# olivesgatech/R3D

Measured on AMD Instinct MI355X. Metric: training clips/sec (RGB+Depth fusion, DARai) at 1/2/4/8 GPUs; effective-rank match, higher is better.
Workload: dtype f32 (depth products: bf16x3 split on the bf16 matrix cores, fp32 accumulate)

## Files before the change

### include/r3d_hip.h

```cpp
#ifndef R3D_HIP_H
#define R3D_HIP_H

#include <stdint.h>

#ifdef __cplusplus
extern "C" {
#endif

#define R3D_ABI_VERSION 2

#define R3D_OK 0
#define R3D_EINVAL (-1)
#define R3D_EALIGN (-2)
#define R3D_ENORCCL (-3)
#define R3D_ERCCL_BASE (-100)

int r3d_abi_version(void);
int r3d_build_info(char* buf, int cap);

int r3d_allreduce_flat(float* buf, int64_t count, void* comm, void* stream);

#define R3D_GEMM_NT 0
#define R3D_GEMM_NN 1
#define R3D_GEMM_TN 2
// ... 97 lines not shown
    const float* q; int32_t ldq; const float* k; int32_t ldk; const float* v; int32_t ldv;
    const uint8_t* key_padding_mask; const int64_t* key_label; int32_t pad_idx;
    float* probs; const uint8_t* drop_mask; float drop_scale; float* o; int32_t ldo;
    int32_t B, heads, Lq, Lk, dh;
} r3d_mha_job;
int r3d_gemm_ln_mha_supported(int heads, int Lq, int Lk, int dh);
int r3d_gemm_ln_mha_fwd(const r3d_gemm_ln_job* jobs, int njobs, int H, const r3d_mha_job* mha, void* stream);

typedef struct r3d_fuser_chain_fwd_args {
    const float* x0; const float* h1;
    const float* wv; const float* wproj; const float* bproj; const float* g2; const float* be2;
    const float* w1; const float* b1; const float* w2; const float* b2; const float* gf; const float* bef;
    const float* pos; const float* wkv; const float* bkv; const float* wseg; const float* bseg;
    float* vsw; float* x1; float* h2; float* m2; float* r2; float* u; float* f1; float* x3; float* y; float* mf; float* rf;
    float* fused; float* seg; float* cakv;
    const float* qpos; const float* w_in; const float* b_in; const float* w_out; const float* b_out; const float* g1;
    const float* be1; const float* wq; const float* bq;
    const uint8_t* drop_sa; const uint8_t* drop_d1; float drop_scale;
    float* sa_qkv; float* p_sa; float* sa_o; float* t1_pre; float* t1; float* m1; float* r1; float* caq;
    int32_t N, S, K, H, add_xres, B, Q, heads;
    uint64_t* timeline;
    const uint16_t* pl_wv; const uint16_t* pl_wproj; const uint16_t* pl_w1; const uint16_t* pl_w2; const uint16_t* pl_wkv;
    const uint16_t* pl_wseg;
} r3d_fuser_chain_fwd_args;
typedef struct r3d_plane_job {
    const float* src; uint16_t* dst; int32_t ld, N, K, transposed, first_block, pad_;
} r3d_plane_job;
int64_t r3d_weight_plane_elems(int N, int K);
int r3d_weight_planes(const r3d_plane_job* jobs_device, int njobs, int total_blocks, void* stream);
int r3d_fuser_chain_supported(int N, int H, int K, int B, int Q, int heads);
int r3d_fuser_chain_fwd(const r3d_fuser_chain_fwd_args* a, void* stream);
typedef struct r3d_fuser_chain_bwd_args {
    const float* d_cakv; const float* d_seg; const float* d_extra; const float* wkv; const float* wseg;
    const float* x3; const float* mf; const float* rf; const float* gf;
    const float* w2; const float* u; const float* w1; const float* x1; const float* m2; const float* r2; const float* g2;
    const float* wproj; const float* wv; const float* x0; const float* m1; const float* r1; const float* g1n;
    const uint8_t* drop_x0; const float* m_rgb; const float* m_dep; const float* rgb; const float* dep_pre;
    const float* mean_d; const float* rstd_d; const float* lnd_g; const float* lnd_b;
    float* d_fused; float* d_x3; float* d_u; float* d_h2; float* d_x1; float* d_v; float* d_h1; float* d_rgb_pre;
    float* d_dep_pre; float* part_nf; float* part_n2; float* part_n1; float* part_dep;
    const float* d_caq; const float* d_t1_res; const float* wq; const float* t1_pre; const float* m1d; const float* r1d;
    const float* g1d; const uint8_t* drop_d1; const float* w_out; const float* sa_qkv; const float* p_sa;
    const uint8_t* drop_sa; const float* w_in;
    float* caqin; float* t1pre_out; float* sap; float* sao; float* saqkv; float* sain; float* part_d1;
    float drop_scale;
    int32_t N, S, K, H, add_xres, B, Q, heads;
// ... 200 lines not shown
```

### r3d_amd/_lib.py

```python
import ctypes as C
import os

HERE = os.path.dirname(os.path.abspath(__file__))
LIB_PATH = os.path.join(HERE, "_build", "libr3d_hip.so")
ABI_VERSION = 2

c_float_p = C.c_void_p


class GemmDesc(C.Structure):
    _fields_ = [
        ("A", C.c_void_p), ("B", C.c_void_p), ("C", C.c_void_p),
        ("layout", C.c_int32), ("M", C.c_int32), ("N", C.c_int32), ("K", C.c_int32),
        ("lda", C.c_int32), ("ldb", C.c_int32), ("ldc", C.c_int32),
        ("a_add", C.c_void_p), ("a_add_mod", C.c_int32), ("a_add_ld", C.c_int32), ("a_row_xor", C.c_int32),
        ("b_add", C.c_void_p), ("b_add_mod", C.c_int32), ("b_add_ld", C.c_int32),
        ("bias", C.c_void_p),
        ("pre_out", C.c_void_p), ("ldpre", C.c_int32),
        ("act", C.c_int32),
        ("drop_mask", C.c_void_p), ("lddrop", C.c_int32), ("drop_scale", C.c_float),
        ("aux", C.c_void_p), ("ldaux", C.c_int32), ("mul", C.c_int32),
        ("res1", C.c_void_p), ("ldr1", C.c_int32),
        ("res2", C.c_void_p), ("ldr2", C.c_int32),
        ("alpha", C.c_float), ("accumulate", C.c_int32),
# ... 21 lines not shown
                ("beta", C.c_void_p), ("relu", C.c_int32), ("add1", C.c_void_p), ("ldadd1", C.c_int32), ("add2", C.c_void_p),
                ("ldadd2", C.c_int32), ("dx", C.c_void_p), ("lddx", C.c_int32), ("dx2", C.c_void_p), ("lddx2", C.c_int32),
                ("drop_mask", C.c_void_p), ("lddrop", C.c_int32), ("drop_scale", C.c_float), ("dgamma", C.c_void_p),
                ("dbeta", C.c_void_p), ("ws", C.c_void_p), ("rows", C.c_int32), ("H", C.c_int32),
                ("rows_per_block", C.c_int32), ("nblocks", C.c_int32)]


class GemmLnJob(C.Structure):
    _fields_ = [("A", C.c_void_p), ("lda", C.c_int32), ("W", C.c_void_p), ("ldw", C.c_int32), ("bias", C.c_void_p),
                ("drop_mask", C.c_void_p), ("lddrop", C.c_int32), ("drop_scale", C.c_float),
                ("res1", C.c_void_p), ("ldr1", C.c_int32), ("res2", C.c_void_p), ("ldr2", C.c_int32),
                ("pre_out", C.c_void_p), ("ldpre", C.c_int32), ("gamma", C.c_void_p), ("beta", C.c_void_p),
                ("y", C.c_void_p), ("ldy", C.c_int32), ("mean", C.c_void_p), ("rstd", C.c_void_p),
                ("pair_out", C.c_void_p), ("M", C.c_int32), ("K", C.c_int32)]


class FuserChainFwdArgs(C.Structure):
    _PTRS = ("x0 h1 wv wproj bproj g2 be2 w1 b1 w2 b2 gf bef pos wkv bkv wseg bseg vsw x1 h2 m2 r2 u f1 x3 y mf rf fused seg "
             "cakv qpos w_in b_in w_out b_out g1 be1 wq bq drop_sa drop_d1").split()
    _PTRS2 = "sa_qkv p_sa sa_o t1_pre t1 m1 r1 caq".split()
    _PLANES = "pl_wv pl_wproj pl_w1 pl_w2 pl_wkv pl_wseg".split()
    _fields_ = ([(n, C.c_void_p) for n in _PTRS] + [("drop_scale", C.c_float)] + [(n, C.c_void_p) for n in _PTRS2] +
                [(n, C.c_int32) for n in "N S K H add_xres B Q heads".split()] + [("timeline", C.c_void_p)] +
                [(n, C.c_void_p) for n in _PLANES])


class PlaneJob(C.Structure):
    _fields_ = [("src", C.c_void_p), ("dst", C.c_void_p), ("ld", C.c_int32), ("N", C.c_int32), ("K", C.c_int32),
                ("transposed", C.c_int32), ("first_block", C.c_int32), ("pad_", C.c_int32)]


class FuserChainBwdArgs(C.Structure):
    _PTRS = ("d_cakv d_seg d_extra wkv wseg x3 mf rf gf w2 u w1 x1 m2 r2 g2 wproj wv x0 m1 r1 g1n drop_x0 m_rgb m_dep rgb "
             "dep_pre mean_d rstd_d lnd_g lnd_b d_fused d_x3 d_u d_h2 d_x1 d_v d_h1 d_rgb_pre d_dep_pre part_nf part_n2 "
             "part_n1 part_dep d_caq d_t1_res wq t1_pre m1d r1d g1d drop_d1 w_out sa_qkv p_sa drop_sa w_in caqin t1pre_out "
             "sap sao saqkv sain part_d1").split()
    _PLANES = "pl_wkv_t pl_wseg_t pl_w2_t pl_w1_t pl_wproj_t pl_wv_t".split()
    _fields_ = ([(n, C.c_void_p) for n in _PTRS] + [("drop_scale", C.c_float)] +
                [(n, C.c_int32) for n in "N S K H add_xres B Q heads".split()] + [("timeline", C.c_void_p)] +
                [(n, C.c_void_p) for n in _PLANES])


class DecoderChainArgs(C.Structure):
    _PTRS = ("caq cakv key_label p_ca drop_ca ca_o wo bo drop_d2 t1 t2_pre g2 be2 t2 m2 r2 w1 b1 drop_ff ff1 w2 b2 drop_d3 "
             "t3_pre d_t3pre d_ff2 d_ff1 d_t2pre d_cap d_cao d_caq d_cakv part_d2").split()
    _fields_ = ([(n, C.c_void_p) for n in _PTRS] + [("drop_scale", C.c_float)] +
                [(n, C.c_int32) for n in "pad_idx B S H Q heads phases".split()] + [("timeline", C.c_void_p)] +
# ... 208 lines not shown
```

### r3d_amd/csrc/chain_common.h

```cpp
#pragma once
#include "common.h"

namespace r3d {

#define R3D_CHAIN_MARK(TL, WG_OK, K) do { if ((TL) && (WG_OK) && threadIdx.x == 0) (TL)[(K)] = wall_clock64(); } while (0)

struct FcMaskSrc {
    const uint8_t* p; size_t ld; bool on;
    __device__ __forceinline__ FcMaskSrc(const uint8_t* m, const void* fallback, size_t ld_)
        : p(m ? m : reinterpret_cast<const uint8_t*>(fallback)), ld(m ? ld_ : 0), on(m != nullptr) {}
    __device__ __forceinline__ uint8_t raw(size_t row, int col) const { return p[row * ld + (on ? col : 0)]; }
    __device__ __forceinline__ float keep(uint8_t b, float scale) const { return on ? scale * (float)b : 1.f; }
};

typedef float f32x4 __attribute__((ext_vector_type(4)));

constexpr int kFcH = 128;
constexpr int kFcRows = 16;
constexpr int kFcP1 = kFcH + 4;
constexpr int kFcP4 = 4 * kFcH + 4;
constexpr int kFcWP = kFcH + 4;
constexpr float kFcEps = 1e-5f;
__device__ __forceinline__ float fc_row16_sum(float v) {
    v += dpp_mov_f<0x128>(v);
// ... 107 lines not shown
#pragma unroll
    for (int i = 0; i < NR; ++i) { sa[i] = fc_row16_sum(a[i]); sb[i] = fc_row16_sum(b[i]); }
    if (li == 0) {
#pragma unroll
        for (int i = 0; i < NR; ++i) {
            red[(0 * 8 + wave) * kFcRows + NR * q + i] = sa[i];
            red[(1 * 8 + wave) * kFcRows + NR * q + i] = sb[i];
        }
    }
    __syncthreads();
#pragma unroll
    for (int i = 0; i < NR; ++i) {
        float x = 0.f, y = 0.f;
#pragma unroll
        for (int w8 = 0; w8 < 8; ++w8) {
            x += red[(0 * 8 + w8) * kFcRows + NR * q + i];
            y += red[(1 * 8 + w8) * kFcRows + NR * q + i];
        }
        sa[i] = x * (1.0f / (float)kFcH);
        sb[i] = y * (1.0f / (float)kFcH);
    }
}

}
```

### r3d_amd/csrc/fuser_chain.hip

```cpp
#include "chain_bf3.h"
#include "mha_small.h"
#include "../../include/r3d_hip.h"

namespace r3d {

constexpr int kFcBufH = 0;
constexpr int kFcBufV = kFcBufH + kFcRows * kFcP1;
constexpr int kFcBufF = kFcBufV + kFcRows * kFcP1;
constexpr int kFcWl = kFcBufF + kFcRows * kFcP4;
constexpr int kFcRed = kFcWl + 8 * 16 * kFcWP;
constexpr int kFcLdsFloats = kFcRed + 2 * 8 * kFcRows;
constexpr int kFcLdsBytes = kFcLdsFloats * 4;
static_assert(mha_small_lds_floats(16, 8) <= 16 * kFcWP, "the query role's attention units borrow the wave's weight region");
static_assert(mha_small_bwd_lds_floats(16, 8) <= 16 * kFcWP, "the query role's attention units borrow the wave's weight region");

typedef r3d_fuser_chain_fwd_args FcFwd;

__device__ __forceinline__ void fc_fwd_fuser(const FcFwd& A, const int wg, float* lds) {
    const int tid = threadIdx.x, lane = tid & 63, wave = tid >> 6;
    const int li = lane & 15, q = lane >> 4;
    float* bufH = lds + kFcBufH;
    float* bufV = lds + kFcBufV;
    float* bufF = lds + kFcBufF;
    float* wl = lds + kFcWl + wave * (16 * kFcWP);
// ... 307 lines not shown
        const int r = 4 * q + i;
        const float t1 = (t1p[i] - mean[i]) * rstd[i] * g1 + be1;
        A.t1[(size_t)(row0 + r) * H + c] = t1;
        bufH[r * kFcP1 + c] = t1 + qp[i];
        if (wave == 0 && li == 0) { A.m1[row0 + r] = mean[i]; A.r1[row0 + r] = rstd[i]; }
    }
    __syncthreads();
    R3D_CHAIN_MARK(A.timeline, wgq == 0, 20);
    fc_opload(a, bufH + li * kFcP1 + 4 * q);
    acc0 = zero; acc1 = zero;
    fc_chunk(a, wr, acc0, acc1);
#pragma unroll
    for (int i = 0; i < 4; ++i) A.caq[(size_t)(row0 + 4 * q + i) * H + c] = (acc0[i] + acc1[i]) + b_q;
    R3D_CHAIN_MARK(A.timeline, wgq == 0, 21);
}

constexpr int kF3P1 = kFcH + 8;
constexpr int kF3P4 = 4 * kFcH + 8;
constexpr int kF3ImgH = 0;
constexpr int kF3ImgV = kF3ImgH + 3 * 16 * kF3P1;
constexpr int kF3ImgF = kF3ImgV + 3 * 16 * kF3P1;
constexpr int kF3RedBytes = (kF3ImgF + 3 * 16 * kF3P4) * 2;
constexpr int kF3LdsBytes = kF3RedBytes + 2 * 2 * 8 * kFcRows * 4;

__device__ __forceinline__ void fc3_fwd_fuser(const FcFwd& A, const int wg, float* lds) {
    const int tid = threadIdx.x, lane = tid & 63, wave = tid >> 6;
    const int li = lane & 15, q = lane >> 4;
    unsigned short* img = reinterpret_cast<unsigned short*>(lds);
    unsigned short* imgH = img + kF3ImgH;
    unsigned short* imgV = img + kF3ImgV;
    unsigned short* imgF = img + kF3ImgF;
    float (*red)[8][kFcRows] = reinterpret_cast<float (*)[8][kFcRows]>(reinterpret_cast<unsigned char*>(lds) + kF3RedBytes);
    const int row0 = wg * kFcRows;
    const int c = wave * 16 + li;
    constexpr int H = kFcH;
    const int nseg_t = (A.K + 15) >> 4;
    const bool has12 = wave < nseg_t;
    R3D_CHAIN_MARK(A.timeline, wg == 0, 0);
    Bf3B b0, b1, b2;
    bf3_bload<4>(b0, A.pl_wv, 4, wave, 0, lane);
    bf3_bload<4>(b1, A.pl_wproj, 4, wave, 0, lane);
    bf3_bload<4>(b2, A.pl_w1, 4, 4 * wave + 0, 0, lane);
    const f32x4 a_in = *reinterpret_cast<const f32x4*>(A.h1 + (size_t)(row0 + (tid >> 5)) * H + 4 * (tid & 31));
    float x0[4];
#pragma unroll
    for (int i = 0; i < 4; ++i) x0[i] = A.x0[(size_t)(row0 + 4 * q + i) * H + c];
// ... 120 lines not shown
    acc0 = zero; acc1 = zero;
    bf3_chunk<4>(imgV, kF3P1, li, q, 0, b1, acc0, acc1);
    if (q >= 2) {
#pragma unroll
        for (int i = 0; i < 4; ++i) A.cakv[(size_t)(fr + i) * (2 * H) + wave * 16 + li] = (acc0[i] + acc1[i]) + bkv0;
    }
    acc0 = zero; acc1 = zero;
    bf3_chunk<4>(imgV, kF3P1, li, q, 0, b2, acc0, acc1);
    if (q >= 2) {
#pragma unroll
        for (int i = 0; i < 4; ++i) A.cakv[(size_t)(fr + i) * (2 * H) + (wave + 8) * 16 + li] = (acc0[i] + acc1[i]) + bkv1;
    }
    if (has12) {
        acc0 = zero; acc1 = zero;
        bf3_chunk<4>(imgV, kF3P1, li, q, 0, b0, acc0, acc1);
        if (q < 2 && cseg < A.K) {
#pragma unroll
            for (int i = 0; i < 4; ++i) A.seg[(size_t)(fr + i) * A.K + cseg] = (acc0[i] + acc1[i]) + bsg;
        }
    }
    R3D_CHAIN_MARK(A.timeline, wg == 0, 7);
}

__global__ __launch_bounds__(512) void fuser_chain_fwd_bf3_kernel(const FcFwd A) {
    extern __shared__ __attribute__((aligned(16))) float lds[];
    if (threadIdx.x >= 256) __builtin_amdgcn_s_setprio(0); else __builtin_amdgcn_s_setprio(2);
    const int nf = (2 * A.N) / kFcRows;
    if ((int)blockIdx.x < nf) fc3_fwd_fuser(A, (int)blockIdx.x, lds);
    else fc_fwd_query(A, (int)blockIdx.x - nf, lds);
}

__global__ __launch_bounds__(256) void weight_planes_kernel(const r3d_plane_job* __restrict__ jobs, int njobs, int total) {
    weight_planes_block(jobs, njobs, total, (int)blockIdx.x * 4 + (threadIdx.x >> 6), threadIdx.x & 63);
}

__global__ __launch_bounds__(512) void fuser_chain_fwd_kernel(const FcFwd A) {
    extern __shared__ __attribute__((aligned(16))) float lds[];
    if (threadIdx.x >= 256) __builtin_amdgcn_s_setprio(0); else __builtin_amdgcn_s_setprio(2);
    const int nf = (2 * A.N) / kFcRows;
    if ((int)blockIdx.x < nf) fc_fwd_fuser(A, (int)blockIdx.x, lds);
    else fc_fwd_query(A, (int)blockIdx.x - nf, lds);
}


constexpr int kFbWl = kFcBufF + kFcRows * kFcP4;
constexpr int kFbRed = kFbWl + 8 * 128 * kFbWP;
constexpr int kFbLdsFloats = kFbRed + 2 * 2 * 8 * kFcRows;
constexpr int kFbLdsBytes = kFbLdsFloats * 4;
static_assert(mha_small_bwd_lds_floats(16, 8) <= 128 * kFbWP, "attention units borrow the wave's weight region");
static_assert(kFbLdsBytes <= 160 * 1024, "LDS");

typedef r3d_fuser_chain_bwd_args FcBwd;
// ... 636 lines not shown

R3D_EXPORT int r3d_fuser_chain_supported(int N, int H, int K, int B, int Q, int heads) {
    return (H == r3d::kFcH && N > 0 && (2 * N) % r3d::kFcRows == 0 && K > 0 && K <= 128 && B > 0 && Q == 8 && heads == 8 &&
            (B * Q) % r3d::kFcRows == 0) ? 1 : 0;
}

R3D_EXPORT int r3d_fuser_chain_fwd(const r3d_fuser_chain_fwd_args* a, void* stream) {
    R3D_REQUIRE(a);
    R3D_REQUIRE(r3d_fuser_chain_supported(a->N, a->H, a->K, a->B, a->Q, a->heads));
    R3D_REQUIRE(a->S > 0 && a->N % a->S == 0);
    R3D_REQUIRE(a->x0 && a->h1 && a->wv && a->wproj && a->bproj && a->g2 && a->be2 && a->w1 && a->b1 && a->w2 && a->b2 && a->gf &&
                a->bef && a->pos && a->wkv && a->bkv && a->wseg && a->bseg);
    R3D_REQUIRE(a->vsw && a->x1 && a->h2 && a->m2 && a->r2 && a->u && a->f1 && a->x3 && a->mf && a->rf && a->fused && a->seg &&
                a->cakv);
    R3D_REQUIRE(a->qpos && a->w_in && a->b_in && a->w_out && a->b_out && a->g1 && a->be1 && a->wq && a->bq);
    R3D_REQUIRE(a->sa_qkv && a->p_sa && a->sa_o && a->t1_pre && a->t1 && a->m1 && a->r1 && a->caq);
    const void* al[] = {a->h1, a->wv, a->wproj, a->w1, a->w2, a->wkv, a->wseg, a->qpos, a->w_in, a->w_out, a->wq, a->sa_o,
                        a->sa_qkv};
    for (const void* p : al)
        if (!r3d_aligned16(p)) return R3D_EALIGN;
    hipError_t e = hipFuncSetAttribute((const void*)r3d::fuser_chain_fwd_kernel, hipFuncAttributeMaxDynamicSharedMemorySize,
                                       r3d::kFcLdsBytes);
    if (e != hipSuccess) return (int)e;
    const int grid = (2 * a->N) / r3d::kFcRows + (a->B * a->Q) / r3d::kFcRows;
    if (a->pl_wv) {
        R3D_REQUIRE(a->pl_wproj && a->pl_w1 && a->pl_w2 && a->pl_wkv && a->pl_wseg);
        const int ldsb = r3d::kFcLdsBytes > r3d::kF3LdsBytes ? r3d::kFcLdsBytes : r3d::kF3LdsBytes;
        e = hipFuncSetAttribute((const void*)r3d::fuser_chain_fwd_bf3_kernel, hipFuncAttributeMaxDynamicSharedMemorySize, ldsb);
        if (e != hipSuccess) return (int)e;
        hipLaunchKernelGGL(r3d::fuser_chain_fwd_bf3_kernel, dim3(grid), dim3(512), (size_t)ldsb, (hipStream_t)stream, *a);
        R3D_LAUNCH_CHECK();
        return R3D_OK;
    }
    hipLaunchKernelGGL(r3d::fuser_chain_fwd_kernel, dim3(grid), dim3(512), (size_t)r3d::kFcLdsBytes, (hipStream_t)stream, *a);
    R3D_LAUNCH_CHECK();
    return R3D_OK;
}

R3D_EXPORT int64_t r3d_weight_plane_elems(int N, int K) { return N > 0 && K > 0 ? (int64_t)r3d::bf3_plane_elems(N, K) : 0; }

R3D_EXPORT int r3d_weight_planes(const r3d_plane_job* jobs_device, int njobs, int total_blocks, void* stream) {
    R3D_REQUIRE(jobs_device && njobs > 0 && total_blocks > 0);
    hipLaunchKernelGGL(r3d::weight_planes_kernel, dim3(r3d_cdiv(total_blocks, 4)), dim3(256), 0, (hipStream_t)stream, jobs_device,
                       njobs, total_blocks);
    R3D_LAUNCH_CHECK();
    return R3D_OK;
}
// ... 33 lines not shown
```

### r3d_amd/engine.py

```python
import math

import torch

from . import ops
from ._lib import GEMM_NT, GEMM_NN, GEMM_TN

LIVE_PREFIXES = ("input_embed.", "depth_projection.", "depth_layernorm.", "pos_embedding", "query_embed.",
                 "fuser.blocks.", "fuser.norm.", "transformer.decoder.", "fc_seg.", "fc.", "fc_len.")
EXCLUDE_CLASS_IDX = 47
DROP_P = 0.1


BN_LIVE_PREFIXES = ("fuser.alpha", "fuser.bn_rgb.", "fuser.bn_depth.")
VARY_LIVE_PREFIXES = ("fuser.alpha",)


def is_live(name):
    return name.startswith(LIVE_PREFIXES)


BWD_BF3_MAX_K = 32


def fuser_chain_shape_ok(B, S, H, K, Q, heads, bn=False):
    return bool(not bn and H // heads == 16 and ops.fuser_chain_supported(B * S, H, K, B, Q, heads))


def decoder_chain_shape_ok(B, S, H, Q, heads, L):
    return bool(L == 1 and H // heads == 16 and B * Q <= 1024 and ops.decoder_chain_supported(H, Q, heads, S))


def bwd_chain_bf3(chain_bf3, K):
    return bool(chain_bf3 and K <= BWD_BF3_MAX_K)


def tail_in_decoder_chain(B, H, K, Q):
    return ops.tail_losses_supported(H, K + 1, Q, B * Q)


class ParamArena:

    def __init__(self, named_params, device, extra_live=()):
        named = list(named_params)
        self.is_live = lambda n: is_live(n) or (bool(extra_live) and n.startswith(tuple(extra_live)))
        live = [(n, p) for n, p in named if self.is_live(n)]
        dead = [(n, p) for n, p in named if not self.is_live(n)]

        def key(item):
# ... 51 lines not shown


class _Shape:

    def __init__(self, eng, B, S, train):
        dev, H, Q, K, L, heads = eng.device, eng.H, eng.Q, eng.K, eng.L, eng.heads
        N, BQ = B * S, B * Q
        f = lambda *s: torch.empty(*s, dtype=torch.float32, device=dev)
        self.B, self.S, self.N, self.BQ = B, S, N, BQ
        self.rgb, self.dep, self.dep_pre = f(N, H), f(N, H), f(N, H)
        self.mean_d, self.rstd_d = f(N), f(N)
        if eng.bn:
            self.bn_mean, self.bn_rstd, self.bn_absg = f(2, H), f(2, H), f(2, H)
            self.bn_idx = torch.empty(2, max(1, int(H * 0.1)), dtype=torch.int64, device=dev)
        self.no_xres = bool(eng.bn or eng.vary)
        self.sums = torch.empty(2, H, dtype=torch.float64, device=dev)
        self.idx = torch.empty(2, H // 4, dtype=torch.int64, device=dev)
        self.mask = f(2, H)
        self.x0, self.h1, self.vsw, self.x1, self.h2 = f(2 * N, H), f(2 * N, H), f(2 * N, H), f(2 * N, H), f(2 * N, H)
        self.u, self.f1 = f(2 * N, 4 * H), f(2 * N, 4 * H)
        self.x3, self.y = f(2 * N, H), f(2 * N, H)
        self.m1, self.r1, self.m2, self.r2, self.mf, self.rf = f(2 * N), f(2 * N), f(2 * N), f(2 * N), f(2 * N), f(2 * N)
        self.fused = f(N, H)
        self.tgt0 = torch.zeros(BQ, H, dtype=torch.float32, device=dev)
        self.layers = []
        for _ in range(L):
            d = dict(sa_qkv=f(BQ, 3 * H), sa_o=f(BQ, H), p_sa=f(B, heads, Q, Q), t1_pre=f(BQ, H),
                     t1=f(BQ, H), m1=f(BQ), r1=f(BQ), caq=f(BQ, H), cakv=f(N, 2 * H), ca_o=f(BQ, H),
                     p_ca=f(B, heads, Q, S), t2_pre=f(BQ, H), t2=f(BQ, H), m2=f(BQ), r2=f(BQ), ff1=f(BQ, 4 * H),
                     t3_pre=f(BQ, H), t3=f(BQ, H), m3=f(BQ), r3=f(BQ))
            self.layers.append(d)
        self.tgtF, self.mF, self.rF = f(BQ, H), f(BQ), f(BQ)
        self.actdur = f(BQ, K + 1)
        self.seg = f(N, K)
        self.loss = f(4)
        self.tables = {}
        self.loss_ws = torch.zeros(ops.losses_ws_floats(B, S, eng.Q), dtype=torch.float32, device=dev)
        self.counts = torch.zeros(4, dtype=torch.int64, device=dev)
        if train:
            self.d_actdur, self.d_seg = torch.zeros(BQ, K + 1, dtype=torch.float32, device=dev), f(N, K)
            self.d_tgtF, self.d_t = f(BQ, H), f(BQ, H)
            self.glayers = [dict(t3pre=f(BQ, H), ff2=f(BQ, H), ff1=f(BQ, 4 * H), t2=f(BQ, H), t2pre=f(BQ, H), cap=f(BQ, H),
                                 cao=f(BQ, H), caq=f(BQ, H), cakv=f(N, 2 * H), caqin=f(BQ, H), t1pre=f(BQ, H), sap=f(BQ, H),
                                 sao=f(BQ, H), saqkv=f(BQ, 3 * H), sain=f(BQ, H), t2b=f(BQ, H)) for _ in range(L)]
            self.d_fused, self.d_fused2 = f(N, H), f(N, H)
            lnw = lambda rows: f(max(ops.layernorm_bwd_ws_floats(rows, H), 4))
# ... 33 lines not shown
        self.pad_idx = module.src_pad_idx
        self.P, self.D = module.depth_projection.in_features, module.input_embed.in_features
        assert self.H % 8 == 0 and self.H % self.heads == 0
        self.bn = hasattr(module.fuser, "bn_rgb")
        self.vary = (not self.bn) and hasattr(module.fuser, "alpha")
        extra = BN_LIVE_PREFIXES if self.bn else (VARY_LIVE_PREFIXES if self.vary else ())
        self.arena = ParamArena(list(module.named_parameters()), self.device, extra)
        self.ws = ops.GemmWorkspace(self.device)
        self._sel = {}
        self.ws_side = ops.GemmWorkspace(self.device)
        self.side = torch.cuda.Stream(self.device)
        self.side2 = torch.cuda.Stream(self.device)
        self.ws_side2 = ops.GemmWorkspace(self.device)
        self.auto_side_stream = True
        self.use_side_stream = False
        self.use_fused_decoder = False
        self.use_fused_tail = True
        self.defer_tail = False
        self.use_paired_launches = True
        self.use_gemm_ln = True
        self.use_fuser_chain = True
        self.use_decoder_chain = True
        self.chain_bf3 = True
        self._planes = None
        self.overlap_planes = False
        self.overlap_param_tail = False
        self.ride_planes = True
        self._planes_rode = False
        self.fuse_depth_adamw = True
        self.pair_embeddings = True
        self._planes_forked = False
        self._tail_pending = False
        self._overlap_tail_now = False
        self.defer_loss_reduce = False
        self.loss_acc = None
        self.fold_rowsums = True
        self.ride_attention = True
        self.ride_attention_bwd = False
        self.split_k4h = False
        self.depth_prec = 1
        self.use_fused_embed = not (self.bn or self.vary)
        self.dropout_enabled = bool(getattr(module, "r3d_dropout_enabled", True))
        self.erank_weight = 0.0
        self.erank_warm_start = False
        self.erank_max_sweeps = 16
        self.erank_side_stream = True
# ... 337 lines not shown
                ent["pl_" + k] = (w_, False)
                ent["pl_" + k + "_t"] = (w_, True)
            self._planes = ops.WeightPlanes(ent, self.device)
        return self._planes

    def _multi_stream(self):
        return bool(self.use_side_stream or (self.auto_side_stream and self.H >= 512 and self.tp is None and
                                             self.grad_hook is None))

    def _planes_refresh(self):
        if self._planes_forked:
            torch.cuda.current_stream().wait_stream(self.side)
            self._planes_forked = False
        elif self._planes_rode:
            pass
        else:
            self.chain_planes().refresh()

    def _join_tail(self):
        if self._tail_pending:
            torch.cuda.current_stream().wait_stream(self.side)
            self._tail_pending = False

    def _chain_shape_ok(self, w):
        return fuser_chain_shape_ok(w.B, w.S, self.H, self.K, self.Q, self.heads, self.bn)

    def _chain_ok(self, w):
        return bool(self.use_fuser_chain and self._chain_shape_ok(w))

    def _dec_chain_ok(self, w):
        return bool(self.use_decoder_chain and decoder_chain_shape_ok(w.B, w.S, self.H, self.Q, self.heads, self.L))

    def _dec_chain(self, w, drop):
        bf3 = bool(self.chain_bf3)
        key = ("dec_chain", bool(drop), bf3)
        if bf3 and not (self.use_fuser_chain and self._chain_shape_ok(w)):
            self._planes_refresh()
        if key not in w.tables:
            pls = self.chain_planes() if bf3 else None
            dpl = None
            if pls is not None:
                dpl = dict(pl_wo=pls.ptr("pl_dec_wo"), pl_w1=pls.ptr("pl_dec_w1"), pl_w2=pls.ptr("pl_dec_w2"),
                           pl_w2_t=pls.ptr("pl_dec_w2_t"), pl_w1_t=pls.ptr("pl_dec_w1_t"), pl_wo_t=pls.ptr("pl_dec_wo_t"))
            a, H = self.arena, self.H
            c, pl = w.layers[0], "transformer.decoder.layers.0."
            dk = (lambda k: w.drop[k]) if drop else (lambda k: None)
# ... 17 lines not shown
        a, H, Q, S, B, BQ, heads, dh = self.arena, self.H, self.Q, w.S, w.B, w.BQ, self.heads, self.dh
        c, pl = w.layers[0], "transformer.decoder.layers.0."
        if self._chain_ok(w):
            bf3 = bool(self.chain_bf3)
            key = ("fwd_chain", bool(drop), bf3)
            if bf3:
                self._planes_refresh()
            if key not in w.tables:
                pls = self.chain_planes() if bf3 else None
                wi, bi = a.p(pl + "multihead_attn.in_proj_weight"), a.p(pl + "multihead_attn.in_proj_bias")
                w.tables[key] = ops.FuserChainFwd(
                    x0=w.x0, h1=w.h1, wv=wv, wproj=a.p(pre + "attn.proj.weight"), bproj=a.p(pre + "attn.proj.bias"),
                    g2=a.p(pre + "norm2.weight"), be2=a.p(pre + "norm2.bias"), w1=a.p(pre + "mlp.mlp.0.weight"),
                    b1=a.p(pre + "mlp.mlp.0.bias"), w2=a.p(pre + "mlp.mlp.2.weight"), b2=a.p(pre + "mlp.mlp.2.bias"),
                    gf=a.p("fuser.norm.weight"), bef=a.p("fuser.norm.bias"), pos=pos.contiguous(), wkv=wi[H:], bkv=bi[H:],
                    wseg=a.p("fc_seg.weight"), bseg=a.p("fc_seg.bias"), vsw=w.vsw, x1=w.x1, h2=w.h2, m2=w.m2, r2=w.r2, u=w.u,
                    f1=w.f1, x3=w.x3, y=w.y, mf=w.mf, rf=w.rf, fused=w.fused, seg=w.seg, cakv=c["cakv"],
                    qpos=qpos, w_in=a.p(pl + "self_attn.in_proj_weight"), b_in=a.p(pl + "self_attn.in_proj_bias"),
                    w_out=a.p(pl + "self_attn.out_proj.weight"), b_out=a.p(pl + "self_attn.out_proj.bias"),
                    g1=a.p(pl + "norm1.weight"), be1=a.p(pl + "norm1.bias"), wq=wi[:H], bq=bi[:H],
                    drop_sa=dm("sa_p0"), drop_d1=dm("d1_0"), drop_scale=dsc, sa_qkv=c["sa_qkv"], p_sa=c["p_sa"],
                    sa_o=c["sa_o"], t1_pre=c["t1_pre"], t1=c["t1"], m1=c["m1"], r1=c["r1"], caq=c["caq"],
                    N=w.N, S=S, K=self.K, H=H, add_xres=0 if w.no_xres else 1, B=B, Q=Q, heads=heads,
                    planes={k: pls.ptr(k) for k in pls.keys if not k.endswith("_t") and "dec_" not in k} if pls is not None else None)
            w.tables[key].launch()
            self._erank_fork(w)
            return
        key = ("fwd_pairs", bool(drop))
        if key not in w.tables:
            wi, bi = a.p(pl + "multihead_attn.in_proj_weight"), a.p(pl + "multihead_attn.in_proj_bias")
            t = 1 if H < 256 else 2
            g1 = ops.GemmGroup(GEMM_NT, [
                dict(a=w.h1, b=wv, c=w.vsw, c_row_xor=1),
                dict(a=w.tgt0, b=a.p(pl + "self_attn.in_proj_weight"), c=c["sa_qkv"], a_add=qpos, a_add_mod=Q,
                     bias=a.p(pl + "self_attn.in_proj_bias"))], tile=t)
            g2 = ops.GemmGroup(GEMM_NT, [
                dict(a=w.h2, b=a.p(pre + "mlp.mlp.0.weight"), c=w.f1, bias=a.p(pre + "mlp.mlp.0.bias"), act=2, pre_out=w.u),
                dict(a=c["sa_o"], b=a.p(pl + "self_attn.out_proj.weight"), c=c["t1_pre"],
                     bias=a.p(pl + "self_attn.out_proj.bias"), drop_mask=self._dm2(dm("d1_0"), BQ, H), drop_scale=dsc)],
                tile=t)
            g3 = ops.GemmGroup(GEMM_NT, [
                dict(a=w.fused, b=a.p("fc_seg.weight"), c=w.seg, bias=a.p("fc_seg.bias")),
                dict(a=w.fused, b=wi[H:], c=c["cakv"], bias=bi[H:], a_add=pos, a_add_mod=S),
                dict(a=c["t1"], b=wi[:H], c=c["caq"], a_add=qpos, a_add_mod=Q, bias=bi[:H])], tile=t)
            w.tables[key] = (g1, g2, g3)
        g1, g2, g3 = w.tables[key]
        g1.launch()
# ... 725 lines not shown
```

### r3d_amd/ops.py

```python
import ctypes as C

import torch

from . import _lib
from ._lib import GemmDesc, GEMM_NT, GEMM_NN, GEMM_TN, check


def _stream():
    return C.c_void_p(torch.cuda.current_stream().cuda_stream)


def _pv(t):
    return None if t is None else t.data_ptr()


def _p(t):
    if t is None:
        return None
    assert t.is_cuda, "r3d_amd kernels take device tensors only"
    return C.c_void_p(t.data_ptr())


def _f32(t, name="tensor"):
    assert t.dtype == torch.float32 and t.is_cuda, f"{name} must be a float32 device tensor"
# ... 342 lines not shown

    def refresh(self):
        check(_lib.load().r3d_weight_planes(_p(self.jobs_dev), self.njobs, self.blocks, _stream()), "r3d_weight_planes")

    def ptr(self, key):
        return self._ptr[key]

    def view(self, key):
        return self._view[key]


class FuserChainFwd:

    def __init__(self, **t):
        from ._lib import FuserChainFwdArgs
        a = FuserChainFwdArgs()
        dims = {k: t.pop(k) for k in ("N", "S", "K", "H", "add_xres", "B", "Q", "heads")}
        a.drop_scale = float(t.pop("drop_scale", 1.0))
        opt = {"y", "drop_sa", "drop_d1"}
        planes = t.pop("planes", None)
        if planes is not None:
            for name in FuserChainFwdArgs._PLANES:
                setattr(a, name, planes[name])
        for name in FuserChainFwdArgs._PTRS + FuserChainFwdArgs._PTRS2:
            v = t.pop(name, None)
            if v is None:
                assert name in opt, name
                continue
            assert v.is_cuda and v.is_contiguous(), name
            assert v.dtype == (torch.uint8 if name.startswith("drop_") else torch.float32), name
            setattr(a, name, v.data_ptr())
        assert not t, t.keys()
        for k, v in dims.items():
            setattr(a, k, int(v))
        self.args = a

    def launch(self):
        check(_lib.load().r3d_fuser_chain_fwd(C.byref(self.args), _stream()), "r3d_fuser_chain_fwd")


class FuserChainBwd:

    def __init__(self, **t):
        from ._lib import FuserChainBwdArgs
        a = FuserChainBwdArgs()
        dims = {k: t.pop(k) for k in ("N", "S", "K", "H", "add_xres", "B", "Q", "heads")}
# ... 604 lines not shown
```

Baseline: 44460.

## Split fuser-chain forward tiles across workgroup groups with last-arriver completion

When the tile grid leaves compute units idle, each 16-row fuser tile is split across 2 or 4 workgroups. Each workgroup computes its slice of the MLP hidden layer (w1) and publishes the bf16x3 planes to a global buffer. The last workgroup to arrive on an atomic counter then runs the w2 product, layernorm, fused and kv/seg outputs alone. This raises parallelism in the widest GEMM for small batches. In exchange it duplicates the early stages (v, proj, LN) in every group, adds global traffic for the packed planes, and adds an atomic handshake.

```diff
diff --git a/include/r3d_hip.h b/include/r3d_hip.h
--- a/include/r3d_hip.h
+++ b/include/r3d_hip.h
@@ -143,6 +143,7 @@
     uint64_t* timeline;
     const uint16_t* pl_wv; const uint16_t* pl_wproj; const uint16_t* pl_w1; const uint16_t* pl_w2; const uint16_t* pl_wkv;
     const uint16_t* pl_wseg;
+    int32_t groups; uint32_t* fc_count; uint64_t* fc_planes;
 } r3d_fuser_chain_fwd_args;
 typedef struct r3d_plane_job {
     const float* src; uint16_t* dst; int32_t ld, N, K, transposed, first_block, pad_;
diff --git a/r3d_amd/_lib.py b/r3d_amd/_lib.py
--- a/r3d_amd/_lib.py
+++ b/r3d_amd/_lib.py
@@ -67,7 +67,7 @@
     _PLANES = "pl_wv pl_wproj pl_w1 pl_w2 pl_wkv pl_wseg".split()
     _fields_ = ([(n, C.c_void_p) for n in _PTRS] + [("drop_scale", C.c_float)] + [(n, C.c_void_p) for n in _PTRS2] +
                 [(n, C.c_int32) for n in "N S K H add_xres B Q heads".split()] + [("timeline", C.c_void_p)] +
-                [(n, C.c_void_p) for n in _PLANES])
+                [(n, C.c_void_p) for n in _PLANES] + [("groups", C.c_int32), ("fc_count", C.c_void_p), ("fc_planes", C.c_void_p)])
 
 
 class PlaneJob(C.Structure):
diff --git a/r3d_amd/csrc/chain_common.h b/r3d_amd/csrc/chain_common.h
--- a/r3d_amd/csrc/chain_common.h
+++ b/r3d_amd/csrc/chain_common.h
@@ -153,4 +153,16 @@
     }
 }
 
+__device__ __forceinline__ bool fc_group_arrive(unsigned* count, int tile, int G, int* flag) {
+    asm volatile("s_waitcnt vmcnt(0)" ::: "memory");
+    __syncthreads();
+    if (threadIdx.x == 0)
+        *flag = (__hip_atomic_fetch_add(count + tile, 1u, __ATOMIC_RELAXED, __HIP_MEMORY_SCOPE_AGENT) == (unsigned)(G - 1)) ? 1 : 0;
+    __syncthreads();
+    return *flag != 0;
 }
+__device__ __forceinline__ void fc_group_reset(unsigned* count, int tile) {
+    if (threadIdx.x == 0) __hip_atomic_store(count + tile, 0u, __ATOMIC_RELAXED, __HIP_MEMORY_SCOPE_AGENT);
+}
+
+}
diff --git a/r3d_amd/csrc/fuser_chain.hip b/r3d_amd/csrc/fuser_chain.hip
--- a/r3d_amd/csrc/fuser_chain.hip
+++ b/r3d_amd/csrc/fuser_chain.hip
@@ -353,6 +353,7 @@
 constexpr int kF3ImgF = kF3ImgV + 3 * 16 * kF3P1;
 constexpr int kF3RedBytes = (kF3ImgF + 3 * 16 * kF3P4) * 2;
 constexpr int kF3LdsBytes = kF3RedBytes + 2 * 2 * 8 * kFcRows * 4;
+static_assert(kF3LdsBytes + 4 <= kFcLdsBytes, "the split's arrival flag sits behind the bf16x3 layout, inside the launch's LDS");
 
 __device__ __forceinline__ void fc3_fwd_fuser(const FcFwd& A, const int wg, float* lds) {
     const int tid = threadIdx.x, lane = tid & 63, wave = tid >> 6;
@@ -519,12 +520,203 @@
     R3D_CHAIN_MARK(A.timeline, wg == 0, 7);
 }
 
+template <int NT>
+__device__ __forceinline__ void fcs_fwd_load(Bf3B& b, const FcFwd& A, int c, int g, int wave, bool has12, int lane) {
+    if (c == 0) bf3_bload<4>(b, A.pl_wv, 4, wave, 0, lane);
+    else if (c == 1) bf3_bload<4>(b, A.pl_wproj, 4, wave, 0, lane);
+    else if (c < 2 + NT) bf3_bload<4>(b, A.pl_w1, 4, 8 * NT * g + NT * wave + (c - 2), 0, lane);
+    else if (c < 6 + NT) bf3_bload<4>(b, A.pl_w2, 16, wave, 4 * (c - 2 - NT), lane);
+    else if (c == 6 + NT) bf3_bload<4>(b, A.pl_wkv, 4, wave, 0, lane);
+    else if (c == 7 + NT) bf3_bload<4>(b, A.pl_wkv, 4, wave + 8, 0, lane);
+    else if (c == 8 + NT) bf3_bload<4>(b, A.pl_wseg, 4, has12 ? wave : 0, 0, lane);
+}
+template <int NT>
+__device__ __forceinline__ void fcs_fwd_step(const unsigned short* img, int pitch, int s0, int c, Bf3B& b0, Bf3B& b1, Bf3B& b2,
+                                             f32x4& acc0, f32x4& acc1, const FcFwd& A, int g, int wave, bool has12, int li,
+                                             int q, int lane) {
+    Bf3B& b = (c % 3 == 0) ? b0 : (c % 3 == 1) ? b1 : b2;
+    bf3_chunk<4>(img, pitch, li, q, s0, b, acc0, acc1);
+    __builtin_amdgcn_sched_barrier(0);
+    fcs_fwd_load<NT>(b, A, c + 3, g, wave, has12, lane);
+    __builtin_amdgcn_sched_barrier(0);
+}
+
+template <int G>
+__device__ __forceinline__ void fc3_fwd_fuser_split(const FcFwd& A, const int tile, const int g, float* lds) {
+    constexpr int NT = 4 / G;
+    const int tid = threadIdx.x, lane = tid & 63, wave = tid >> 6;
+    const int li = lane & 15, q = lane >> 4;
+    unsigned short* img = reinterpret_cast<unsigned short*>(lds);
+    unsigned short* imgH = img + kF3ImgH;
+    unsigned short* imgV = img + kF3ImgV;
+    unsigned short* imgF = img + kF3ImgF;
+    float (*red)[8][kFcRows] = reinterpret_cast<float (*)[8][kFcRows]>(reinterpret_cast<unsigned char*>(lds) + kF3RedBytes);
+    int* flag = reinterpret_cast<int*>(reinterpret_cast<unsigned char*>(lds) + kF3LdsBytes);
+    const int row0 = tile * kFcRows;
+    const int c = wave * 16 + li;
+    constexpr int H = kFcH;
+    const int nseg_t = (A.K + 15) >> 4;
+    const bool has12 = wave < nseg_t;
+    const bool lead = g == 0;
+    R3D_CHAIN_MARK(A.timeline, tile == 0 && lead, 0);
+    Bf3B b0, b1, b2;
+    fcs_fwd_load<NT>(b0, A, 0, g, wave, has12, lane);
+    fcs_fwd_load<NT>(b1, A, 1, g, wave, has12, lane);
+    fcs_fwd_load<NT>(b2, A, 2, g, wave, has12, lane);
+    const f32x4 a_in = *reinterpret_cast<const f32x4*>(A.h1 + (size_t)(row0 + (tid >> 5)) * H + 4 * (tid & 31));
+    float x0[4];
+#pragma unroll
+    for (int i = 0; i < 4; ++i) x0[i] = A.x0[(size_t)(row0 + 4 * q + i) * H + c];
+    const float b_proj = A.bproj[c], g2 = A.g2[c], be2 = A.be2[c], b_2 = A.b2[c], gF = A.gf[c], beF = A.bef[c];
+    const int ft0 = 8 * NT * g + NT * wave;
+    float b_1[NT];
+#pragma unroll
+    for (int t = 0; t < NT; ++t) b_1[t] = A.b1[(ft0 + t) * 16 + li];
+    const int f0 = (row0 >> 1) + 2 * q;
+    const float pos0 = A.pos[(size_t)(f0 % A.S) * H + c], pos1 = A.pos[(size_t)((f0 + 1) % A.S) * H + c];
+    const float bkv0 = A.bkv[wave * 16 + li], bkv1 = A.bkv[(wave + 8) * 16 + li];
+    const int cseg = (has12 ? wave : 0) * 16 + li;
+    const float bsg = A.bseg[cseg < A.K ? cseg : A.K - 1];
+    __builtin_amdgcn_sched_barrier(0);
+    bf3_stage_tile(imgH, kF3P1, 0, a_in, tid);
+    __syncthreads();
+    R3D_CHAIN_MARK(A.timeline, tile == 0 && lead, 1);
+    const f32x4 zero = {0.f, 0.f, 0.f, 0.f};
+    f32x4 acc0 = zero, acc1 = zero;
+    fcs_fwd_step<NT>(imgH, kF3P1, 0, 0, b0, b1, b2, acc0, acc1, A, g, wave, has12, li, q, lane);
+#pragma unroll
+    for (int i = 0; i < 4; ++i) {
+        const float v = acc0[i] + acc1[i];
+        const int rs = 4 * q + (i ^ 1);
+        if (lead) A.vsw[(size_t)(row0 + rs) * H + c] = v;
+        bf3_store1(imgV, kF3P1, rs, c, v);
+    }
+    __syncthreads();
+    R3D_CHAIN_MARK(A.timeline, tile == 0 && lead, 2);
+    acc0 = zero; acc1 = zero;
+    fcs_fwd_step<NT>(imgV, kF3P1, 0, 1, b0, b1, b2, acc0, acc1, A, g, wave, has12, li, q, lane);
+    float x1[4], mean[4], rstd[4];
+#pragma unroll
+    for (int i = 0; i < 4; ++i) {
+        x1[i] = (acc0[i] + acc1[i]) + b_proj + x0[i];
+        if (lead) A.x1[(size_t)(row0 + 4 * q + i) * H + c] = x1[i];
+    }
+    fc_layernorm(x1, red, wave, li, q, mean, rstd);
+#pragma unroll
+    for (int i = 0; i < 4; ++i) {
+        const float h = (x1[i] - mean[i]) * rstd[i] * g2 + be2;
+        const int r = 4 * q + i;
+        if (lead) A.h2[(size_t)(row0 + r) * H + c] = h;
+        bf3_store1(imgH, kF3P1, r, c, h);
+        if (lead && wave == 0 && li == 0) { A.m2[row0 + r] = mean[i]; A.r2[row0 + r] = rstd[i]; }
+    }
+    __syncthreads();
+    R3D_CHAIN_MARK(A.timeline, tile == 0 && lead, 3);
+#pragma unroll
+    for (int t = 0; t < NT; ++t) {
+        acc0 = zero; acc1 = zero;
+        fcs_fwd_step<NT>(imgH, kF3P1, 0, 2 + t, b0, b1, b2, acc0, acc1, A, g, wave, has12, li, q, lane);
+        const int cu = (ft0 + t) * 16 + li;
+#pragma unroll
+        for (int i = 0; i < 4; ++i) {
+            const float u = (acc0[i] + acc1[i]) + b_1[t];
+            const float f = gelu_f(u);
+            const size_t o = (size_t)(row0 + 4 * q + i) * (4 * H) + cu;
+            A.u[o] = u;
+            A.f1[o] = f;
+            unsigned short hh, mm, ll;
+            bf3_split1(f, hh, mm, ll);
+            __hip_atomic_store(reinterpret_cast<unsigned long long*>(A.fc_planes) + o,
+                               (unsigned long long)hh | ((unsigned long long)mm << 16) | ((unsigned long long)ll << 32),
+                               __ATOMIC_RELAXED, __HIP_MEMORY_SCOPE_AGENT);
+        }
+    }
+    R3D_CHAIN_MARK(A.timeline, tile == 0 && lead, 4);
+    if (!fc_group_arrive(A.fc_count, tile, G, flag)) return;
+    fc_group_reset(A.fc_count, tile);
+    {
+        const int r = tid >> 5, c4 = tid & 31;
+        const unsigned long long* pp =
+            reinterpret_cast<const unsigned long long*>(A.fc_planes) + (size_t)(row0 + r) * (4 * H) + 4 * c4;
+        unsigned long long v[4][4];
+#pragma unroll
+        for (int k = 0; k < 4; ++k)
+#pragma unroll
+            for (int e = 0; e < 4; ++e) v[k][e] = __hip_atomic_load(pp + 128 * k + e, __ATOMIC_RELAXED, __HIP_MEMORY_SCOPE_AGENT);
+#pragma unroll
+        for (int k = 0; k < 4; ++k) {
+            unsigned short* dst = imgF + r * kF3P4 + 128 * k + 4 * c4;
+#pragma unroll
+            for (int pl = 0; pl < 3; ++pl)
+                *reinterpret_cast<uint2*>(dst + pl * 16 * kF3P4) =
+                    make_uint2(((unsigned)(v[k][0] >> (16 * pl)) & 0xffffu) | (((unsigned)(v[k][1] >> (16 * pl)) & 0xffffu) << 16),
+                               ((unsigned)(v[k][2] >> (16 * pl)) & 0xffffu) | (((unsigned)(v[k][3] >> (16 * pl)) & 0xffffu) << 16));
+        }
+    }
+    __syncthreads();
+    R3D_CHAIN_MARK(A.timeline, tile == 0, 8);
+    acc0 = zero; acc1 = zero;
+#pragma unroll
+    for (int j = 0; j < 4; ++j)
+        fcs_fwd_step<NT>(imgF, kF3P4, 4 * j, 2 + NT + j, b0, b1, b2, acc0, acc1, A, g, wave, has12, li, q, lane);
+    R3D_CHAIN_MARK(A.timeline, tile == 0, 5);
+    float x3[4];
+#pragma unroll
+    for (int i = 0; i < 4; ++i) {
+        x3[i] = (acc0[i] + acc1[i]) + b_2 + x1[i] + (A.add_xres ? x0[i] : 0.f);
+        A.x3[(size_t)(row0 + 4 * q + i) * H + c] = x3[i];
+    }
+    fc_layernorm(x3, red, wave, li, q, mean, rstd);
+    float y[4];
+#pragma unroll
+    for (int i = 0; i < 4; ++i) {
+        y[i] = (x3[i] - mean[i]) * rstd[i] * gF + beF;
+        if (A.y) A.y[(size_t)(row0 + 4 * q + i) * H + c] = y[i];
+        if (wave == 0 && li == 0) { A.mf[row0 + 4 * q + i] = mean[i]; A.rf[row0 + 4 * q + i] = rstd[i]; }
+    }
+    {
+        const float fu0 = (y[0] + y[1]) * 0.5f, fu1 = (y[2] + y[3]) * 0.5f;
+        A.fused[(size_t)f0 * H + c] = fu0;
+        A.fused[(size_t)(f0 + 1) * H + c] = fu1;
+        bf3_store1(imgV, kF3P1, 2 * q, c, fu0);
+        bf3_store1(imgV, kF3P1, 2 * q + 1, c, fu1);
+        bf3_store1(imgV, kF3P1, 8 + 2 * q, c, fu0 + pos0);
+        bf3_store1(imgV, kF3P1, 8 + 2 * q + 1, c, fu1 + pos1);
+    }
+    __syncthreads();
+    R3D_CHAIN_MARK(A.timeline, tile == 0, 6);
+    const int fr = (row0 >> 1) + ((4 * q) & 7);
+    acc0 = zero; acc1 = zero;
+    fcs_fwd_step<NT>(imgV, kF3P1, 0, 6 + NT, b0, b1, b2, acc0, acc1, A, g, wave, has12, li, q, lane);
+    if (q >= 2) {
+#pragma unroll
+        for (int i = 0; i < 4; ++i) A.cakv[(size_t)(fr + i) * (2 * H) + wave * 16 + li] = (acc0[i] + acc1[i]) + bkv0;
+    }
+    acc0 = zero; acc1 = zero;
+    fcs_fwd_step<NT>(imgV, kF3P1, 0, 7 + NT, b0, b1, b2, acc0, acc1, A, g, wave, has12, li, q, lane);
+    if (q >= 2) {
+#pragma unroll
+        for (int i = 0; i < 4; ++i) A.cakv[(size_t)(fr + i) * (2 * H) + (wave + 8) * 16 + li] = (acc0[i] + acc1[i]) + bkv1;
+    }
+    if (has12) {
+        acc0 = zero; acc1 = zero;
+        fcs_fwd_step<NT>(imgV, kF3P1, 0, 8 + NT, b0, b1, b2, acc0, acc1, A, g, wave, has12, li, q, lane);
+        if (q < 2 && cseg < A.K) {
+#pragma unroll
+            for (int i = 0; i < 4; ++i) A.seg[(size_t)(fr + i) * A.K + cseg] = (acc0[i] + acc1[i]) + bsg;
+        }
+    }
+    R3D_CHAIN_MARK(A.timeline, tile == 0, 7);
+}
+
 __global__ __launch_bounds__(512) void fuser_chain_fwd_bf3_kernel(const FcFwd A) {
     extern __shared__ __attribute__((aligned(16))) float lds[];
     if (threadIdx.x >= 256) __builtin_amdgcn_s_setprio(0); else __builtin_amdgcn_s_setprio(2);
-    const int nf = (2 * A.N) / kFcRows;
-    if ((int)blockIdx.x < nf) fc3_fwd_fuser(A, (int)blockIdx.x, lds);
-    else fc_fwd_query(A, (int)blockIdx.x - nf, lds);
+    const int nf = (2 * A.N) / kFcRows, G = A.groups > 1 ? A.groups : 1, b = (int)blockIdx.x;
+    if (b >= nf * G) fc_fwd_query(A, b - nf * G, lds);
+    else if (G == 4) fc3_fwd_fuser_split<4>(A, b >> 2, b & 3, lds);
+    else if (G == 2) fc3_fwd_fuser_split<2>(A, b >> 1, b & 1, lds);
+    else fc3_fwd_fuser(A, b, lds);
 }
 
 __global__ __launch_bounds__(256) void weight_planes_kernel(const r3d_plane_job* __restrict__ jobs, int njobs, int total) {
@@ -1207,7 +1399,9 @@
     hipError_t e = hipFuncSetAttribute((const void*)r3d::fuser_chain_fwd_kernel, hipFuncAttributeMaxDynamicSharedMemorySize,
                                        r3d::kFcLdsBytes);
     if (e != hipSuccess) return (int)e;
-    const int grid = (2 * a->N) / r3d::kFcRows + (a->B * a->Q) / r3d::kFcRows;
+    const int G = a->groups > 1 ? a->groups : 1;
+    R3D_REQUIRE(a->groups <= 1 || ((a->groups == 2 || a->groups == 4) && a->pl_wv && a->fc_count && a->fc_planes));
+    const int grid = (2 * a->N) / r3d::kFcRows * G + (a->B * a->Q) / r3d::kFcRows;
     if (a->pl_wv) {
         R3D_REQUIRE(a->pl_wproj && a->pl_w1 && a->pl_w2 && a->pl_wkv && a->pl_wseg);
         const int ldsb = r3d::kFcLdsBytes > r3d::kF3LdsBytes ? r3d::kFcLdsBytes : r3d::kF3LdsBytes;
diff --git a/r3d_amd/engine.py b/r3d_amd/engine.py
--- a/r3d_amd/engine.py
+++ b/r3d_amd/engine.py
@@ -24,6 +24,14 @@
 
 def fuser_chain_shape_ok(B, S, H, K, Q, heads, bn=False):
     return bool(not bn and H // heads == 16 and ops.fuser_chain_supported(B * S, H, K, B, Q, heads))
+
+
+def fuser_chain_groups(B, S, Q, n_cu):
+    tiles, nq = (2 * B * S) // 16, (B * Q) // 16
+    for g in (4, 2):
+        if tiles * g + nq <= n_cu:
+            return g
+    return 1
 
 
 def decoder_chain_shape_ok(B, S, H, Q, heads, L):
@@ -121,6 +129,9 @@
         self.x3, self.y = f(2 * N, H), f(2 * N, H)
         self.m1, self.r1, self.m2, self.r2, self.mf, self.rf = f(2 * N), f(2 * N), f(2 * N), f(2 * N), f(2 * N), f(2 * N)
         self.fused = f(N, H)
+        self.fc_groups = eng._fc_groups(B, S)
+        self.fc_count = torch.zeros(max(2 * N // 16, 1), dtype=torch.int32, device=dev) if self.fc_groups > 1 else None
+        self.fc_planes = torch.empty(2 * N * 4 * H, dtype=torch.int64, device=dev) if self.fc_groups > 1 else None
         self.tgt0 = torch.zeros(BQ, H, dtype=torch.float32, device=dev)
         self.layers = []
         for _ in range(L):
@@ -200,6 +211,8 @@
         self.use_fuser_chain = True
         self.use_decoder_chain = True
         self.chain_bf3 = True
+        self.fc_groups_force = 0
+        self._n_cu = None
         self._planes = None
         self.overlap_planes = False
         self.overlap_param_tail = False
@@ -583,6 +596,13 @@
             torch.cuda.current_stream().wait_stream(self.side)
             self._tail_pending = False
 
+    def _fc_groups(self, B, S):
+        if self.fc_groups_force:
+            return int(self.fc_groups_force)
+        if self._n_cu is None:
+            self._n_cu = torch.cuda.get_device_properties(self.device).multi_processor_count
+        return fuser_chain_groups(B, S, self.Q, self._n_cu)
+
     def _chain_shape_ok(self, w):
         return fuser_chain_shape_ok(w.B, w.S, self.H, self.K, self.Q, self.heads, self.bn)
 
@@ -646,7 +666,8 @@
                     drop_sa=dm("sa_p0"), drop_d1=dm("d1_0"), drop_scale=dsc, sa_qkv=c["sa_qkv"], p_sa=c["p_sa"],
                     sa_o=c["sa_o"], t1_pre=c["t1_pre"], t1=c["t1"], m1=c["m1"], r1=c["r1"], caq=c["caq"],
                     N=w.N, S=S, K=self.K, H=H, add_xres=0 if w.no_xres else 1, B=B, Q=Q, heads=heads,
-                    planes={k: pls.ptr(k) for k in pls.keys if not k.endswith("_t") and "dec_" not in k} if pls is not None else None)
+                    planes={k: pls.ptr(k) for k in pls.keys if not k.endswith("_t") and "dec_" not in k} if pls is not None else None,
+                    groups=w.fc_groups if bf3 else 1, fc_count=w.fc_count, fc_planes=w.fc_planes)
             w.tables[key].launch()
             self._erank_fork(w)
             return
diff --git a/r3d_amd/ops.py b/r3d_amd/ops.py
--- a/r3d_amd/ops.py
+++ b/r3d_amd/ops.py
@@ -388,6 +388,10 @@
         if planes is not None:
             for name in FuserChainFwdArgs._PLANES:
                 setattr(a, name, planes[name])
+        groups, fc_count, fc_planes = int(t.pop("groups", 1)), t.pop("fc_count", None), t.pop("fc_planes", None)
+        if groups > 1:
+            assert planes is not None and fc_count.dtype == torch.int32 and fc_planes.dtype == torch.int64
+            a.groups, a.fc_count, a.fc_planes = groups, fc_count.data_ptr(), fc_planes.data_ptr()
         for name in FuserChainFwdArgs._PTRS + FuserChainFwdArgs._PTRS2:
             v = t.pop(name, None)
             if v is None:
```

New measurement: 45030 (median of 6 runs). 1.01x the previous value.
